# wagnva/semantic-nerf-for-satellite-data

Measured on AMD Instinct MI355X. Metric: train rays/sec (4096 rays x 64 samples), higher is better.
Workload: dtype f32(f16x2)

## Files before the change

semantic-nerf-for-satellite-data_amd/csrc/api.hip:

```cpp
#include <stdarg.h>
#include <stdio.h>
#include <stdlib.h>
#include <string.h>

#include <mutex>

#include "aux_kernels.h"
#include "bsp.h"
#include "composite.h"
#include "gemm.h"
#include "plan.h"

namespace snerf {

int forward_bsp(const Plan& p, const float* pk, const SnerfInputs* in, const SnerfOutputs* out, void* workspace, hipStream_t st);
int backward_bsp(const Plan& p, const float* pk, const SnerfInputs* in, const SnerfOutGrads* go, float* gp, float* d_t, float* d_t_s,
                 void* workspace, hipStream_t st);

static thread_local char g_err[512] = "";
void set_error(const char* fmt, ...) {
  va_list ap;
  va_start(ap, fmt);
  vsnprintf(g_err, sizeof(g_err), fmt, ap);
  va_end(ap);
// ... 182 lines not shown
  p.FA = p.Wf + p.Xp;
  int nb = 0;
  p.blk_rgb = nb++;
  p.blk_sem = sem ? nb++ : -1;
  p.blk_beta = nb++;
  p.blk_sbeta = sbeta ? nb++ : -1;
  p.blk_sun = nb++;
  p.nblk = nb;
  p.KF = (nb - 1) * p.H;
  p.KF = round_up(p.KF, 128);
  p.sun_col = p.KF;
  p.N1 = p.KF + p.H;

  size_t off = 0;
  auto take = [&](size_t n) { size_t o = off; off += round_up_sz(n, 64); return o; };
  for (int i = 0; i < p.L; ++i) {
    p.k_tr[i] = (i == 0) ? p.Ep : (((p.skip_mask >> i) & 1u) ? p.Ep + p.W : p.W);
    p.w_tr[i] = take((size_t)p.W * p.k_tr[i]);
    p.b_tr[i] = take(p.W);
  }
  p.w_fs = take((size_t)(p.W + NARROW) * p.W); p.b_fs = take(p.W + NARROW);
  p.w_h1 = take((size_t)p.N1 * p.FA); p.b_h1 = take(p.N1);
  p.w_s2 = take((size_t)p.H * p.H); p.b_s2 = take(p.H);
  p.w_s3 = take((size_t)p.H * p.H); p.b_s3 = take(p.H);
  p.w_s4 = take((size_t)NARROW * p.H); p.b_s4 = take(NARROW);
  p.w_fin = take((size_t)NARROW * p.KF); p.b_fin = take(NARROW);
  p.sky_floats = 9 * p.H + 4;
  p.sky = take(p.sky_floats);
  p.n_fp32 = off;
  {
    const char* ev = getenv("SNERF_COMPOSE_FEATS");
    p.compose_feats = p.pl == 2 && (p.H & 31) == 0 && p.N1 + NARROW <= 2048 && !(ev && ev[0] == '0' && ev[1] == 0);
  }
  if (!p.compose_feats) { plan_weights(p); plan_bsp(p); return SNERF_OK; }
  Plan q = p;
  q.compose_feats = false;
  plan_weights(q);
  plan_bsp(q);
  plan_weights(p);
  plan_bsp(p);
  if (q.packed_floats > p.packed_floats) p.packed_floats = q.packed_floats;
  if (q.ws_bytes > p.ws_bytes) p.ws_bytes = q.ws_bytes;
  return SNERF_OK;
}

struct TableBuilder {
  CopyTable tabs[4];
  int nt = 0;
  bool missing = false;
  TableBuilder() { memset(tabs, 0, sizeof(tabs)); nt = 1; }
  void add(float* user, int user_ld, int rows, int cols, size_t dst_off, int dst_ld) {
    if (!user) { missing = true; return; }
    if (tabs[nt - 1].n == COPY_TABLE_MAX) ++nt;
    CopyEntry& e = tabs[nt - 1].e[tabs[nt - 1].n++];
    e.user = user; e.user_ld = user_ld; e.rows = rows; e.cols = cols; e.dst_off = dst_off; e.dst_ld = dst_ld;
  }
};

static void build_tables(const Plan& p, const SnerfParams* w, TableBuilder& tb) {
  const int W = p.W, H = p.H, E = p.E;
  for (int i = 0; i < p.L; ++i) {
    const bool skip = (p.skip_mask >> i) & 1u;
    if (i == 0) {
      tb.add(w->fc_w[0], E, W, E, p.w_tr[0], p.k_tr[0]);
    } else if (skip) {
      tb.add(w->fc_w[i], E + W, W, E, p.w_tr[i], p.k_tr[i]);
// ... 256 lines not shown
```

semantic-nerf-for-satellite-data_amd/csrc/aux_kernels.h:

```cpp
#pragma once
#include "common.h"
#include "../../include/snerf_hip.h"

namespace snerf {

struct EncodeArgs {
  const float* rays = nullptr;
  const float* xyz = nullptr;
  const float* z = nullptr;
  const float* sun_d = nullptr; int sun_stride = 3;
  const float* t = nullptr; const float* t_s = nullptr;
  int dir_is_sun = 0;
  int N = 0, S = 0, F = 0, Ep = 0;
  int FA = 0, W = 0, Xp = 0, x_sun = 0, x_t = 3, x_ts = -1, tau = 0;
  unsigned* zero = nullptr; int zero_n = 0;
};

struct CopyEntry {
  float* user; int user_ld; int rows; int cols; unsigned long long dst_off; int dst_ld;
};
constexpr int COPY_TABLE_MAX = 40;
struct CopyTable { CopyEntry e[COPY_TABLE_MAX]; int n; };

int launch_zero_bytes(void* p, size_t bytes, hipStream_t st);
int launch_sample_z(const float* rays, const float* zsteps, const float* u, float* z, int N, int S, hipStream_t st);
int launch_copy_table(const CopyTable& tb, float* packed, int mode, hipStream_t st);
int launch_reduce_rows(const float* in, int n_in, size_t in_stride, int width, float* out, size_t out_stride,
                       int group, int accumulate, hipStream_t st);
int reduce_partials(const float* in, int n_in, size_t in_stride, int width, float* tmp, float* out, hipStream_t st);
struct RedJob { const float* in; float* out; unsigned long long stride; long long width; int n_in; int blk0; int vec; int cols; int in_ld; int out_ld; int store; int pad; };
constexpr int RED_MAX = 56;
struct RedTable { RedJob j[RED_MAX]; int n = 0; int blocks = 0; };
constexpr int RED_CHUNK = 24;
struct RedChunk { RedJob j[RED_CHUNK]; int n = 0; };
int red_add_elem(RedTable& tb, const float* in, int n_in, size_t stride, size_t width, float* out);
int red_add_elem2d(RedTable& tb, const float* in, int n_in, size_t stride, int rows, int cols, int in_ld, float* out, int out_ld);
int red_add_col(RedTable& tb, const float* in, int n_in, size_t stride, int width, float* out);
int red_store_last(RedTable& tb);
int launch_reductions(const RedTable& elem, const RedTable& col, hipStream_t st);
int launch_ray_sum32(const float* d32, int col0, int N, int S, int tau, float* out, hipStream_t st);
int launch_embedding_rows(const float* table, int n_embed, int tau, const long long* idx, int n, float* rows, hipStream_t st);
int launch_embedding_backward(const long long* idx, const float* d_rows, int n, int tau, int n_embed, float* grad, hipStream_t st);

}
```

semantic-nerf-for-satellite-data_amd/csrc/bsp.h:

```cpp
#pragma once
#include "common.h"
#include "gemm.h"

namespace snerf {
namespace bsp {

constexpr int RB = 128;
constexpr int CB = 128;
constexpr int E_MAX = 100;
constexpr int E_QUIET = 60;

typedef __amdgpu_buffer_rsrc_t srd_t;
typedef unsigned int u32x4 __attribute__((ext_vector_type(4)));
typedef unsigned int u32x2 __attribute__((ext_vector_type(2)));
typedef _Float16 f16x8 __attribute__((ext_vector_type(8)));
typedef _Float16 f16x4 __attribute__((ext_vector_type(4)));
constexpr unsigned OOB = 0xFFFFFFF0u;

__host__ __device__ inline int ncb_of(int ld) { return (ld + CB - 1) / CB; }
__host__ __device__ inline size_t plane_bytes(size_t rows, int ld, int pl = 2) { return rows * (size_t)ld * 2 * pl; }
__host__ __device__ inline size_t etab_ints(size_t rows, int ld) { return ((rows + RB - 1) / RB) * (size_t)ncb_of(ld); }
__host__ __device__ inline unsigned g16_off(int k, int pl = 2) { return (unsigned)(k >> 4) * 32u * (unsigned)pl + (unsigned)(k & 15) * 2u; }

__host__ __device__ inline int exp_of_maxbits(unsigned b) {
// ... 45 lines not shown
}

__device__ __forceinline__ void sum8(const u32x4 hi, const u32x4 lo, float (&x)[8]) {
#pragma unroll
  for (int i = 0; i < 4; ++i) {
    asm("v_fma_mix_f32 %0, %1, 1.0, %2 op_sel_hi:[1,0,1]" : "=v"(x[2 * i]) : "v"(hi[i]), "v"(lo[i]));
    asm("v_fma_mix_f32 %0, %1, 1.0, %2 op_sel:[1,0,1] op_sel_hi:[1,0,1]" : "=v"(x[2 * i + 1]) : "v"(hi[i]), "v"(lo[i]));
  }
}
__device__ __forceinline__ void cvt8f(const u32x4 hi, float (&x)[8]) {
  const f16x8 h = __builtin_bit_cast(f16x8, hi);
#pragma unroll
  for (int i = 0; i < 8; ++i) x[i] = (float)h[i];
}

__host__ __device__ inline int wf16_row(int m) { return (m & 0x13) | ((m & 4) << 1) | ((m & 8) >> 1); }

struct KcArgs {
  const char* A = nullptr; const int* EA = nullptr; int lda = 0; int a_col0 = 0;
  const char* A2 = nullptr; const int* EA2 = nullptr; int lda2 = 0; int a2_col0 = 0;
  int Ka = 0;
  const char* W = nullptr;
  const int* EW = nullptr;
  int w_rb32 = 0, w_row0 = 0, w_k0 = 0; unsigned w_bytes = 0;
  int I = 0, J = 0, K = 0;
  char* C = nullptr; int* EC = nullptr; int ldc = 0; int c_col0 = 0;
  float* Cf = nullptr;
  const float* bias = nullptr;
  int act = ACT_NONE; float w0 = 1.f;
  unsigned* Csign = nullptr;
  int aux_mode = AUX_NONE;
  const char* H = nullptr; const int* EH = nullptr; int ldh = 0; int h_col0 = 0; const unsigned* Hsign = nullptr;
  float* colsum = nullptr; int ldcs = 0;
  int tiles_i = 0, tiles_j = 0;
  int tj_skip = -1;
  int tiles_jr = 0;
  int rev = 0;
  int dbg = 0;
  int* tile_ctr = nullptr;
  int pl = 2;
  const float* nd_w = nullptr; float* nd_out = nullptr; unsigned long long nd_stride = 0;
  int nd_omax = 0, nd_ldw = 0;
  int nd_rows[8] = {0, 0, 0, 0, 0, 0, 0, 0}, nd_row0[8] = {0, 0, 0, 0, 0, 0, 0, 0}, nd_woff[8] = {0, 0, 0, 0, 0, 0, 0, 0};
};
__host__ __device__ inline size_t sign_words(size_t rows, int ld) { return ((rows + 31) / 32) * (size_t)((ld + 63) / 64) * 64; }

struct DwArgs {
  const char* A = nullptr; const int* EA = nullptr; int lda = 0; int a_col0 = 0;
  const char* B = nullptr; const int* EB = nullptr; int ldb = 0; int b_col0 = 0;
  int I = 0, J = 0, P = 0;
  float* C = nullptr; int ldc = 0;
  int k_split = 0, n_split = 1; unsigned long long slab_stride = 0;
  int tiles_i = 0, tiles_j = 0;
  int pl = 2;
};

constexpr int TR_MAXL = 8;
constexpr int TR_SLOTS = TR_MAXL + 1;
struct TrunkArgs {
  const char* pe = nullptr; const int* Epe = nullptr;
  int P = 0, W = 0, L = 0; unsigned skip_mask = 0;
  int gamma_free_layer = 0;
  const char* Wp[TR_SLOTS] = {}; const int* EW[TR_SLOTS] = {}; unsigned w_bytes[TR_SLOTS] = {}; int K[TR_SLOTS] = {};
  const float* bias[TR_SLOTS] = {}; float w0[TR_SLOTS] = {};
  char* F = nullptr; int* EF = nullptr; int ldf = 0;
  char* H[TR_MAXL] = {}; int* EH[TR_MAXL] = {}; unsigned* Hsign[TR_MAXL] = {};
// ... 69 lines not shown
```

semantic-nerf-for-satellite-data_amd/csrc/bsp_aux.hip:

```cpp
#include "bsp.h"
#include "aux_kernels.h"

namespace snerf {
namespace bsp {

__device__ __forceinline__ float block_max_256(float m, float* sm) {
#pragma unroll
  for (int o = 32; o >= 1; o >>= 1) m = fmaxf(m, __shfl_xor(m, o, 64));
  __syncthreads();
  if ((threadIdx.x & 63) == 0) sm[threadIdx.x >> 6] = m;
  __syncthreads();
  return fmaxf(fmaxf(sm[0], sm[1]), fmaxf(sm[2], sm[3]));
}

__global__ __launch_bounds__(256) void to_planes_kernel(const float* __restrict__ src, int ld_src, int rows, int cols,
                                                        char* __restrict__ dst, int* __restrict__ E, int ld, int col0, int pl) {
  __shared__ float sm[4];
  const int rb = blockIdx.y, cb = blockIdx.x;
  const int t = threadIdx.x, c8 = cb * 128 + (t & 15) * 8;
  float v[8][8];
  float m = 0.f;
#pragma unroll
  for (int i = 0; i < 8; ++i) {
    const int r = rb * 128 + (t >> 4) + 16 * i;
// ... 402 lines not shown
    float4 tsum = make_float4(0.f, 0.f, 0.f, 0.f);
#pragma unroll
    for (int i = 0; i < 32; ++i) { const float4 q = sm[i][threadIdx.x]; tsum.x += q.x; tsum.y += q.y; tsum.z += q.z; tsum.w += q.w; }
    *reinterpret_cast<float4*>(partial + (size_t)blockIdx.x * 32 + 4 * threadIdx.x) = tsum;
  }
  if (pl == nullptr) return;
  int e[2];
#pragma unroll
  for (int h = 0; h < 2; ++h) {
    e[h] = exp_of_maxbits(__float_as_uint(smx[0][h]));
    if (threadIdx.x == 0 && r0 + 128 * h < rows) E[(r0 >> 7) + h] = e[h];
  }
#pragma unroll
  for (int i = 0; i < 8; ++i) {
    const int r = r0 + rg + 32 * i;
    if (r >= rows) continue;
    const float sc = pow2f(e[i >> 2]);
    const float x[4] = {v[i].x * sc, v[i].y * sc, v[i].z * sc, v[i].w * sc};
    f16x4 h, l;
#pragma unroll
    for (int c = 0; c < 4; ++c) { h[c] = (_Float16)x[c]; l[c] = (_Float16)(x[c] - (float)h[c]); }
    char* d = pl + (size_t)r * 64 * npl + g16_off(4 * c4, npl);
    *reinterpret_cast<f16x4*>(d) = h;
    if (npl == 2) *reinterpret_cast<f16x4*>(d + 32) = l;
  }
}

int launch_colsum32_bsp(const float* in, int rows, float* partial, char* planes, int* E, int pl, hipStream_t st) {
  hipLaunchKernelGGL(colsum32_bsp_kernel, dim3((rows + 255) / 256), dim3(256), 0, st, in, rows, partial, planes, E, pl);
  SNERF_LAUNCH_CHECK();
  return SNERF_OK;
}

}
}
```

semantic-nerf-for-satellite-data_amd/csrc/bsp_kc.hip:

```cpp
#include "bsp_kc_epi.h"

namespace snerf {
namespace bsp {

constexpr int KC_A = 128 * 128, KC_RING = 3;
constexpr int KC_RINGB = KC_RING * KC_A;
constexpr int KC_XREG = KC_RINGB;
constexpr int KC_BIAS = KC_XREG + 4 * 4096;
constexpr int KC_ETAB = KC_BIAS + 2 * 1024;
constexpr int KC_SMAX = KC_ETAB + 2 * 512;
constexpr int KC_NEXT = KC_SMAX + 64;
constexpr int KC_HSIGN = KC_NEXT + 64;
constexpr int KC_LDS = KC_HSIGN + 4 * 1024;
constexpr int KC_NDW = KC_HSIGN;
constexpr int KC_NDW_FLOATS = 2560;
constexpr int KC_LDS_ND = KC_NDW + 4 * KC_NDW_FLOATS;
template <int PL, int ACT, int AUX, bool COLSUM, bool SIGNS, int SINM, bool DIAG = false, int NDOT = 0>
__global__ __launch_bounds__(256, 2) void gemm_kc_kernel(const KcArgs) {
  const kargs_t p = kargs();
  __shared__ __attribute__((aligned(16))) char lds[NDOT > 0 ? KC_LDS_ND : KC_LDS];
  float* smax = reinterpret_cast<float*>(lds + KC_SMAX);
  const int t = threadIdx.x, lane = t & 63;
  const int wave = __builtin_amdgcn_readfirstlane(t >> 6);
  const int wj0 = wave * 64;
// ... 482 lines not shown
                const unsigned rs = __float_as_uint(root) | ((sword[mi] << (31 - (16 * nj + 8 * gg + c))) & 0x80000000u);
                v[c] *= __uint_as_float(rs);
              }
            } else if (AUX == AUX_RELU_MASK) {
              float hv[8];
              cvt8f(hh[gg], hv);
#pragma unroll
              for (int c = 0; c < 8; ++c) v[c] = hv[c] > 0.f ? v[c] : 0.f;
            }
#pragma unroll
            for (int c = 0; c < 8; ++c) {
              if (COLSUM) cs[8 * gg + c] += v[c];
              acc[mi][nj][8 * gg + c] = v[c];
            }
            if (jw + 16 * gq < e->J) {
              const float m8 = absmax3(v[6], v[7], absmax3(v[4], v[5], absmax3(v[2], v[3], absmax3(v[0], v[1], 0.f))));
              wmax = fmaxf(wmax, (BIAS && (32 * mi + pt) >= nrows) ? 0.f : m8);
            }
          }
        }
        if (COLSUM && e->colsum != nullptr) {
#pragma unroll
          for (int r = 0; r < 16; ++r) cs[r] = sum32(cs[r]);
          if ((el & 31) == 31) {
#pragma unroll
            for (int gg = 0; gg < 2; ++gg)
              if (jw + 16 * (2 * nj + gg) < e->J) {
                float* d = e->colsum + (size_t)c_ti * e->ldcs + jw + 16 * (2 * nj + gg) + 8 * lh;
                *reinterpret_cast<float4*>(d) = make_float4(cs[8 * gg] * fac, cs[8 * gg + 1] * fac, cs[8 * gg + 2] * fac, cs[8 * gg + 3] * fac);
                *reinterpret_cast<float4*>(d + 4) = make_float4(cs[8 * gg + 4] * fac, cs[8 * gg + 5] * fac, cs[8 * gg + 6] * fac, cs[8 * gg + 7] * fac);
              }
          }
        }
      }
      constexpr bool RAW = AUX != AUX_NONE || COLSUM;
      wmax = wave_max(wmax) * (RAW ? fac : 1.f);
      if (el == 0) smax[wave] = wmax;
      barrier_raw();
      const float bmax = fmaxf(smax[wave & 2], smax[(wave & 2) + 1]);
      const int eC = exp_of_maxbits(__float_as_uint(bmax));
      const float sc = pow2f(eC) * (RAW ? fac : 1.f);
      if ((wave & 1) == 0 && el == 0 && wave_cols) e->EC[(size_t)c_ti * ncb_of(e->ldc) + ((e->c_col0 + jw) >> 7)] = eC;
      if (more) headW();
#pragma unroll
      for (int mi = 0; mi < 4; ++mi) {
        u32x4 ph1[4];
#pragma unroll
        for (int nj = 0; nj < 2; ++nj) {
          u32x4 phi[2], plo[2];
#pragma unroll
          for (int gg = 0; gg < 2; ++gg) {
            float v[8];
#pragma unroll
            for (int c = 0; c < 8; ++c) v[c] = acc[mi][nj][8 * gg + c];
            if constexpr (PL == 2) {
              split8(v, sc, phi[gg], plo[gg]);
              strip_put(gg, phi[gg], plo[gg]);
            } else {
              cvt8(v, sc, ph1[2 * nj + gg]);
              strip_put1(nj, gg, ph1[2 * nj + gg]);
            }
          }
          if constexpr (PL == 2) {
            strip_flush(mi, nj);
            keep_planes(phi, plo);
          }
        }
        if constexpr (PL == 1) {
          strip_flush(mi, 0);
          keep_planes1(ph1);
        }
      }
    }
    if (!more) break;
    vb = vbn;
    first = false;
  }
}

int prof_hook_begin(double flops, int variant, hipStream_t st);
void prof_hook_end(int token, hipStream_t st);
int check_kc(const KcArgs& a, bool narrow);

static int g_kc_grid_override = 0;
void kc_set_grid_override(int n) { g_kc_grid_override = n > 0 ? n : 0; }
static int kc_slots() {
  if (g_kc_grid_override > 0) return g_kc_grid_override;
  static const int n = [] {
    int dev = 0, cus = 256;
    if (hipGetDevice(&dev) != hipSuccess || hipDeviceGetAttribute(&cus, hipDeviceAttributeMultiprocessorCount, dev) != hipSuccess || cus <= 0) cus = 256;
    return 2 * cus;
  }();
  return n;
}

static bool cs_bias_check(const KcArgs& a) {
  if (a.colsum != nullptr && a.bias != nullptr) { set_error("bsp gemm: bias and column sums in one launch"); return true; }
  return false;
}

int launch_kc(const KcArgs& a0, hipStream_t st) {
  KcArgs a = a0;
  if (!a.A2) { a.A2 = a.A; a.EA2 = a.EA; a.lda2 = a.lda; a.a2_col0 = a.a_col0; if (a.Ka == 0) a.Ka = a.K; }
  int rc = check_kc(a, false);
  if (rc) return rc;
  if (cs_bias_check(a)) return SNERF_ERR_BAD_DESC;
  a.tiles_i = (a.I + 127) / 128;
  a.tiles_jr = (a.J + 255) / 256;
  if (a.tj_skip >= a.tiles_jr || (a.tj_skip >= 0 && a.tiles_jr < 2)) { set_error("bsp gemm: tj_skip beyond the column tiles"); return SNERF_ERR_BAD_DESC; }
  a.tiles_j = a.tiles_jr - (a.tj_skip >= 0 ? 1 : 0);
  if (a.nd_w != nullptr) {
    if (a.nd_omax == 0) { a.nd_omax = 1; a.nd_ldw = 0; for (int tj = 0; tj < 8; ++tj) { a.nd_rows[tj] = tj < a.tiles_jr ? 1 : 0; a.nd_row0[tj] = 0; } }
    int off = 0;
    for (int tj = 0; tj < a.tiles_jr && tj < 8; ++tj) { a.nd_woff[tj] = off; off += 256 * a.nd_rows[tj]; }
    if (a.tiles_jr > 8 || off > KC_NDW_FLOATS || (a.nd_omax != 1 && a.nd_omax != 5)) { set_error("bsp gemm: folded projections beyond the LDS table"); return SNERF_ERR_BAD_DESC; }
    for (int tj = 0; tj < a.tiles_jr; ++tj) if (a.nd_rows[tj] > a.nd_omax) { set_error("bsp gemm: nd_rows > nd_omax"); return SNERF_ERR_BAD_DESC; }
  }
#ifdef KC_DIAG_BUILD
  constexpr bool DIAG = true;
  static const int dbg = [] { const char* e = getenv("SNERF_KC_DBG"); return e ? atoi(e) : 0; }();
  a.dbg = dbg;
  if (dbg & 2) a.w_bytes = 0;
#else
  constexpr bool DIAG = false;
#endif
  const int ntiles = a.tiles_i * a.tiles_j, slots = kc_slots();
  const dim3 grid(ntiles < slots ? ntiles : slots), block(256);
  const int tok = prof_hook_begin(2.0 * a.I * (double)a.J * a.K, 0, st);
  const bool cs = a.colsum != nullptr;
#define KC_LAUNCH(ACT_, AUX_, CS_, SG_, SM_) do { if (a.pl == 2) hipLaunchKernelGGL((gemm_kc_kernel<2, ACT_, AUX_, CS_, SG_, SM_, DIAG>), grid, block, 0, st, a); \
// ... 24 lines not shown
```

semantic-nerf-for-satellite-data_amd/csrc/bsp_pass.hip:

```cpp
#include "aux_kernels.h"
#include "bsp.h"
#include "composite.h"
#include "normals.h"
#include "plan.h"

namespace snerf {

namespace {
struct Ws {
  char* base;
  char* c(size_t off) const { return base + off; }
  float* f(size_t off) const { return reinterpret_cast<float*>(base + off); }
  int* i(size_t off) const { return reinterpret_cast<int*>(base + off); }
  unsigned* u(size_t off) const { return reinterpret_cast<unsigned*>(base + off); }
  void a(bsp::KcArgs& g, const PlaneT& t, int k, int col0 = 0) const { g.A = c(t.o); g.EA = i(t.e); g.lda = t.ld; g.a_col0 = col0; g.Ka = k; }
  void a2(bsp::KcArgs& g, const PlaneT& t) const { g.A2 = c(t.o); g.EA2 = i(t.e); g.lda2 = t.ld; }
  void out(bsp::KcArgs& g, const PlaneT& t, int col0 = 0) const { g.C = c(t.o); g.EC = i(t.e); g.ldc = t.ld; g.c_col0 = col0; g.Csign = t.s ? u(t.s) : nullptr; }
  void h(bsp::KcArgs& g, const PlaneT& t, int col0 = 0) const { g.H = c(t.o); g.EH = i(t.e); g.ldh = t.ld; g.h_col0 = col0; g.Hsign = t.s ? u(t.s) : nullptr; }
  void dz(bsp::DwArgs& g, const PlaneT& t) const { g.A = c(t.o); g.EA = i(t.e); g.lda = t.ld; g.a_col0 = 0; }
  void x(bsp::DwArgs& g, const PlaneT& t, int col0) const { g.B = c(t.o); g.EB = i(t.e); g.ldb = t.ld; g.b_col0 = col0; }
};
struct WOp { const char* W; const int* EW; int rb32; unsigned bytes; int K; };
WOp wop(const Plan& p, const float* pk, int job) {
  const char* planes = reinterpret_cast<const char*>(pk + p.n_fp32);
// ... 245 lines not shown
    g.k_split = m.sp.k_split; g.n_split = m.sp.ns; g.slab_stride = m.stride; g.pl = p.pl;
    return bsp::launch_dw(g, narrow_i, st);
  };
  auto dw_reduce = [&](const DwMat& m, size_t count, float* gout) { return red_add_elem(rq.elem, m.slab, m.sp.ns, m.stride, count, gout); };
  auto narrow_grad = [&](const float* dnar, float* part, const PlaneT& t, float* gout) {
    RC(bsp::launch_colsum32_bsp(dnar, P, part, ws.c(t.o), ws.i(t.e), p.pl, st));
    return red_add_col(rq.col, part, (P + 255) / 256, NARROW, NARROW, gout);
  };
  float* dsig = ws.f(p.o_dsig); float* dfin = ws.f(p.o_dfin); float* dsun = ws.f(p.o_dsun);
  if (embed && p.sc) {
    if (d_t) RC(launch_zero_bytes(d_t, (size_t)p.N * p.tau * sizeof(float), st));
    if (d_t_s && p.x_ts >= 0) RC(launch_zero_bytes(d_t_s, (size_t)p.N * p.tau * sizeof(float), st));
    return SNERF_OK;
  }
  CompBwdArgs b;
  CompArgs& c = b.f;
  c.N = p.N; c.S = p.S; c.H = H; c.C = p.C; c.sc = p.sc; c.sem_sigmoid = p.sem_sigmoid; c.has_sbeta = p.blk_sbeta >= 0;
  c.z = ws.f(p.o_z); c.sigo = ws.f(p.o_sigo); c.fino = ws.f(p.o_fino); c.suno = ws.f(p.o_suno);
  narrow_parts(c, p, pk, ws);
  c.sun_d = in->sun_d; c.sun_stride = in->sun_stride; c.sky = pk + p.sky;
  b.T = ws.f(p.o_T); b.rgbraw = ws.f(p.o_rgbraw);
  b.g_rgb = go->rgb; b.g_depth = go->depth; b.g_weights = go->weights; b.g_transparency = go->transparency;
  b.g_albedo = go->albedo; b.g_sun = go->sun; b.g_sky = go->sky; b.g_beta = go->beta; b.g_sigmas = go->sigmas;
  b.g_beta_s = go->beta_semantic; b.g_logits = go->semantic_logits;
  b.d_sigo = dsig; b.d_fino = dfin; b.d_suno = dsun; b.sky_slab = (p.sc || embed) ? nullptr : ws.f(p.o_skyslab);
  b.zero = ws.u(p.o_kcq); b.zero_n = KCQ_SLOTS * 16;
  RC(launch_composite_bwd(b, st));
  if (!p.sc && !embed)
    RC(red_add_col(rq.col, ws.f(p.o_skyslab), p.comp_blocks * 4, (size_t)p.sky_floats, p.sky_floats, gp + p.sky));


  const PlaneT dz1 = p.dza.view(p.h1w);
  const int sun_col = p.sc ? 0 : p.sun_col;
  if (!p.sc) {
    if (embed) RC(bsp::launch_colsum32_bsp(dfin, P, r.nar_fin, ws.c(p.pdfin.o), ws.i(p.pdfin.e), p.pl, st));
    else {
      RC(narrow_grad(dfin, r.nar_fin, p.pdfin, gp + p.b_fin));
      RC(dw_gemm(r.w_fin, p.pdfin, NARROW, true, p.h1, 0, p.KF));
      RC(dw_reduce(r.w_fin, (size_t)NARROW * p.KF, gp + p.w_fin));
    }
    bsp::KcArgs g;
    ws.a(g, p.pdfin, NARROW); weights(g, p, pk, p.wj_tfin);
    g.I = P; g.J = p.KF; g.K = NARROW; ws.out(g, dz1);
    dact(g, p.h1);
    colsum(g, r.cs_fin, p.KF);
    if (p.compose_feats) g.ldcs = r.ld_cs1;
    RC(launch_kc(g));
    if (!p.compose_feats && !embed) RC(bias_from_colsum(r.cs_fin, p.KF, gp + p.b_h1));
  }
  if (!embed) {
    RC(narrow_grad(dsun, r.nar_sun, p.pdsun, gp + p.b_s4));
    RC(dw_gemm(r.w_s4, p.pdsun, NARROW, true, p.s3, 0, H));
    RC(dw_reduce(r.w_s4, (size_t)NARROW * H, gp + p.w_s4));
    bsp::KcArgs g;
    ws.a(g, p.pdsun, NARROW); weights(g, p, pk, p.wj_ts4);
    g.I = P; g.J = H; g.K = NARROW; ws.out(g, p.dsa);
    dact(g, p.s3);
    colsum(g, r.cs_s3, H);
    RC(launch_kc(g));
    RC(bias_from_colsum(r.cs_s3, H, gp + p.b_s3));
    RC(dw_gemm(r.w_s3, p.dsa, H, false, p.s2, 0, H));
    RC(dw_reduce(r.w_s3, (size_t)H * H, gp + p.w_s3));
    ws.a(g, p.dsa, H); g.K = H; weights(g, p, pk, p.wj_ts3);
    ws.out(g, p.dsb);
    dact(g, p.s2);
    colsum(g, r.cs_s2, H);
    RC(launch_kc(g));
    RC(bias_from_colsum(r.cs_s2, H, gp + p.b_s2));
    RC(dw_gemm(r.w_s2, p.dsb, H, false, p.h1, sun_col, H));
    RC(dw_reduce(r.w_s2, (size_t)H * H, gp + p.w_s2));
    ws.a(g, p.dsb, H); weights(g, p, pk, p.wj_ts2);
    ws.out(g, dz1, sun_col);
    dact(g, p.h1, sun_col);
    colsum(g, r.cs_sun, H);
    if (p.compose_feats) g.ldcs = r.ld_cs1;
    RC(launch_kc(g));
    if (!p.compose_feats) RC(bias_from_colsum(r.cs_sun, H, gp + p.b_h1 + (size_t)p.sun_col));
  }
  auto transient_grads = [&]() {
    const bool want_t = d_t != nullptr, want_ts = d_t_s != nullptr && p.x_ts >= 0;
    if (p.sc) {
      if (want_t) RC(launch_zero_bytes(d_t, (size_t)p.N * p.tau * sizeof(float), st));
      if (want_ts) RC(launch_zero_bytes(d_t_s, (size_t)p.N * p.tau * sizeof(float), st));
    } else if (want_t || want_ts) {
      int b_lo = p.blk_beta, b_hi = p.blk_beta;
      auto use = [&](int blk, bool on) { if (on && blk >= 0) { if (blk < b_lo) b_lo = blk; if (blk > b_hi) b_hi = blk; } };
      use(p.blk_rgb, p.rgb_t); use(p.blk_sem, p.sem_t || p.sem_ts); use(p.blk_sbeta, true);
      const int k_lo = b_lo * H, k_n = (b_hi + 1 - b_lo) * H;
      float* dext = ws.f(p.o_dfin);
      bsp::KcArgs x;
      ws.a(x, dz1, k_n, k_lo); weights(x, p, pk, p.wj_th1, p.Wf, k_lo);
      x.I = P; x.J = p.Xp; x.K = k_n; x.Cf = dext;
      RC(bsp::launch_kc_narrow(x, st));
      if (want_t) RC(launch_ray_sum32(dext, p.x_t, p.N, p.S, p.tau, d_t, st));
      if (want_ts) RC(launch_ray_sum32(dext, p.x_ts, p.N, p.S, p.tau, d_t_s, st));
    }
    return (int)SNERF_OK;
  };
  if (embed) return transient_grads();
  PlaneT dz_cur = p.dza.view(W);
  PlaneT dz_nxt = p.dzb.view(W);
  const bool sig_live = !p.sc || go->weights != nullptr || go->transparency != nullptr || go->sigmas != nullptr;
  const PlaneT& hl = p.h[p.L - 1];
  bool uncompose = false;
  if (p.compose_feats) {
    const int r0 = p.sc ? p.sun_col : 0;
    const int nt = (P + 127) / 128, X = p.FA - W;
    RC(dw_gemm(r.w_h1, dz1, p.h1w, false, p.fa, 0, p.FA));
    RC(red_add_elem2d(rq.elem, r.w_h1.slab + W, r.w_h1.sp.ns, r.w_h1.stride, p.h1w, X, p.FA, gp + p.w_h1 + (size_t)r0 * p.FA + W, p.FA));
    RC(red_add_elem2d(rq.elem, r.w_h1.slab, r.w_h1.sp.ns, r.w_h1.stride, p.h1w, W, p.FA, r.w_h1.slab, p.FA));
    RC(red_store_last(rq.elem));
    RC(red_add_col(rq.col, r.cs_fin, nt, (size_t)r.ld_cs1, p.h1w, r.cs_fin));
    RC(red_store_last(rq.col));
    uncompose = true;
    RC(transient_grads());
    if (sig_live) {
      RC(narrow_grad(dsig, r.nar_sig, p.pdsig, gp + p.b_fs + W));
      RC(dw_gemm(r.w_fs, p.pdsig, NARROW, true, hl, 0, W));
      RC(dw_reduce(r.w_fs, (size_t)NARROW * W, gp + p.w_fs + (size_t)W * W));
    }
    { const PlaneT sw = dz_cur; dz_cur = dz_nxt; dz_nxt = sw; }
    bsp::KcArgs g;
    ws.a(g, dz1, p.h1w);
    if (sig_live) ws.a2(g, p.pdsig);
    weights(g, p, pk, p.wj_th1, 0, r0); g.I = P; g.J = W; g.K = sig_live ? p.h1w + NARROW : p.h1w;
    ws.out(g, dz_cur);
    dact(g, hl, 0, (p.L == 1) ? 30.f : 1.f);
    colsum(g, r.cs_hl, W);
    RC(launch_kc(g));
    RC(bias_from_colsum(r.cs_hl, W, gp + p.b_tr[p.L - 1]));
  }
  const PlaneT dfa = p.dzb.view(p.FA);
  if (!p.compose_feats) {
    const int r0 = p.sc ? p.sun_col : 0;
    RC(dw_gemm(r.w_h1, dz1, p.h1w, false, p.fa, 0, p.FA));
    RC(dw_reduce(r.w_h1, (size_t)p.h1w * p.FA, gp + p.w_h1 + (size_t)r0 * p.FA));
    bsp::KcArgs g;
    ws.a(g, dz1, p.h1w); weights(g, p, pk, p.wj_th1, 0, r0);
    g.I = P; g.J = W; g.K = p.h1w; ws.out(g, dfa);
    colsum(g, r.cs_fa, p.FA);
    RC(launch_kc(g));
    RC(red_add_col(rq.col, r.cs_fa, (P + 127) / 128, (size_t)cs_ld(p.FA), W, gp + p.b_fs));
    RC(transient_grads());
  }
  if (!p.compose_feats) {
    if (sig_live) RC(narrow_grad(dsig, r.nar_sig, p.pdsig, gp + p.b_fs + W));
    RC(dw_gemm(r.w_fs, dfa, W, false, hl, 0, W));
    if (sig_live) RC(dw_gemm(r.w_fs, p.pdsig, NARROW, true, hl, 0, W, (size_t)W * W));
    RC(dw_reduce(r.w_fs, (size_t)(sig_live ? W + NARROW : W) * W, gp + p.w_fs));
    bsp::KcArgs g;
    ws.a(g, dfa, W);
    if (sig_live) ws.a2(g, p.pdsig);
    weights(g, p, pk, p.wj_tfs); g.I = P; g.J = W; g.K = sig_live ? W + NARROW : W;
    ws.out(g, dz_cur);
    dact(g, hl, 0, (p.L == 1) ? 30.f : 1.f);
    colsum(g, r.cs_hl, W);
    RC(launch_kc(g));
    RC(bias_from_colsum(r.cs_hl, W, gp + p.b_tr[p.L - 1]));
  }
  for (int i = p.L - 1; i >= 0; --i) {
    const BwdRegions::Layer& t = r.tr[i];
    if (i > 0 && ((p.skip_mask >> i) & 1u)) {
      RC(dw_gemm(t.w_gamma, dz_cur, W, false, p.pe, 0, p.Ep));
      RC(dw_gemm(t.w, dz_cur, W, false, p.h[i - 1], 0, W));
      RC(red_add_elem2d(rq.elem, t.w_gamma.slab, t.w_gamma.sp.ns, t.w_gamma.stride, W, p.Ep, p.Ep, gp + p.w_tr[i], p.k_tr[i]));
      RC(red_add_elem2d(rq.elem, t.w.slab, t.w.sp.ns, t.w.stride, W, W, W, gp + p.w_tr[i] + p.Ep, p.k_tr[i]));
    } else {
      if (i == 0) RC(dw_gemm(t.w, dz_cur, W, false, p.pe, 0, p.Ep));
      else RC(dw_gemm(t.w, dz_cur, W, false, p.h[i - 1], 0, W));
      RC(dw_reduce(t.w, (size_t)W * p.k_tr[i], gp + p.w_tr[i]));
    }
    if (i == 0) break;
    bsp::KcArgs g;
    ws.a(g, dz_cur, W); weights(g, p, pk, p.wj_tt[i]);
    g.I = P; g.J = W; g.K = W; ws.out(g, dz_nxt);
    dact(g, p.h[i - 1], 0, (i - 1 == 0) ? 30.f : 1.f);
// ... 80 lines not shown
```

semantic-nerf-for-satellite-data_amd/csrc/plan.h:

```cpp
#pragma once
#include "bsp.h"
#include "common.h"
#include "../../include/snerf_hip.h"

namespace snerf {

constexpr int NARROW = 32;
constexpr int MAX_CLASSES = 16;
constexpr int ND_FIN = 5;
constexpr int MAX_SKY_UNITS = 8;

struct PlaneT { size_t o = 0, e = 0, s = 0; int ld = 0; };
struct PlaneScratch {
  size_t o = 0, e = 0; int maxw = 0;
  PlaneT view(int ld) const { PlaneT t; t.o = o; t.e = e; t.ld = ld; return t; }
};

struct Plan {
  int N = 0, S = 0, P = 0, Pp = 0;
  int W = 0, H = 0, L = 0, E = 0, Ep = 0, F = 0, tau = 0, C = 0;
  bool siren = false, train = false, sc = false, sem_sigmoid = false;
  bool relight = false;
  bool embed_grad = false;
  bool geometry = false;
// ... 14 lines not shown
  size_t w_h1 = 0, b_h1 = 0;
  size_t w_s2 = 0, b_s2 = 0, w_s3 = 0, b_s3 = 0;
  size_t w_s4 = 0, b_s4 = 0;
  size_t w_fin = 0, b_fin = 0;
  size_t sky = 0;
  int sky_floats = 0;
  size_t n_fp32 = 0;
  size_t packed_floats = 0;
  int pl = 2;

  size_t o_z = 0, o_T = 0, o_rgbraw = 0;
  PlaneT pe, fa, h1, s2, s3, h[SNERF_MAX_LAYERS];
  size_t o_sigo = 0, o_fino = 0, o_suno = 0;
  size_t o_sigpart = 0, o_sunpart = 0, o_finpart = 0;
  bool nd_sig = false, nd_sun = false;
  bool fuse_trunk = false;
  bool nd_fin = false;
  PlaneScratch dza, dzb;
  PlaneT dsa, dsb, pdsig, pdfin, pdsun;
  size_t o_dsig = 0, o_dfin = 0, o_dsun = 0;
  size_t o_skyslab = 0;
  size_t o_kcq = 0;
  size_t o_rq = 0, rq_floats = 0;
  bsp::WPackTable wj = {};
  int wj_tr[SNERF_MAX_LAYERS] = {0}, wj_tt[SNERF_MAX_LAYERS] = {0};
  int wj_fs = 0, wj_sig = 0, wj_tfs = 0, wj_h1 = 0, wj_th1 = 0, wj_s2 = 0, wj_ts2 = 0, wj_s3 = 0, wj_ts3 = 0, wj_s4 = 0, wj_ts4 = 0,
      wj_fin = 0, wj_tfin = 0;
  size_t wp_bytes = 0;
  int h1w = 0;
  bool compose_feats = false;
  int wj_first = 0;
  size_t o_wc = 0;
  size_t o_bc = 0;
  int comp_blocks = 0;
  size_t ws_bytes = 0;
};

inline bool skips_beta_block(const Plan& p, bool want_beta) {
  return p.nd_fin && !p.train && p.H == 256 && p.blk_beta >= 0 && !want_beta && !p.rgb_t && p.blk_sbeta < 0;
}

constexpr int KCQ_SLOTS = 64;
struct DwSplit { int ns = 1; int k_split = 32; };
DwSplit dw_choose_bsp(int P, int rows, int cols, bool narrow_rows);

#define RC(expr) do { int _rc = (expr); if (_rc) return _rc; } while (0)

int make_plan(const SnerfDesc* d, Plan* pl);

size_t bsp_rq_floats(const Plan& p);

}
```

Measured before the change: 170,000.

## Compute per-ray extras weight grads and transient grads from 64-row column sums

Since the extra input columns (sun direction, transient embeddings) are constant within each ray, the backward GEMM epilogue now also writes 64-row column sums of the h1 gradient. A new ray_extras kernel uses these sums to build the extras' weight-gradient slab and the d_t/d_t_s gradients. This lets the dW GEMM for the first head layer cover only W columns, and removes the separate transient-gradient GEMM over the full sample count. The cost is an extra epilogue store, a new kernel and stricter shape requirements (S divisible by 64, tau ≤ 16, Xp == 16).

```diff
diff --git a/semantic-nerf-for-satellite-data_amd/csrc/api.hip b/semantic-nerf-for-satellite-data_amd/csrc/api.hip
--- a/semantic-nerf-for-satellite-data_amd/csrc/api.hip
+++ b/semantic-nerf-for-satellite-data_amd/csrc/api.hip
@@ -238,6 +238,10 @@
     const char* ev = getenv("SNERF_COMPOSE_FEATS");
     p.compose_feats = p.pl == 2 && (p.H & 31) == 0 && p.N1 + NARROW <= 2048 && !(ev && ev[0] == '0' && ev[1] == 0);
   }
+  {
+    const char* ev = getenv("SNERF_RAY_EXTRAS");
+    p.ray_extras = p.compose_feats && p.train && p.S % 64 == 0 && ((p.N1 + 3) & ~3) <= 2048 && !(ev && ev[0] == '0' && ev[1] == 0);
+  }
   if (!p.compose_feats) { plan_weights(p); plan_bsp(p); return SNERF_OK; }
   Plan q = p;
   q.compose_feats = false;
diff --git a/semantic-nerf-for-satellite-data_amd/csrc/aux_kernels.h b/semantic-nerf-for-satellite-data_amd/csrc/aux_kernels.h
--- a/semantic-nerf-for-satellite-data_amd/csrc/aux_kernels.h
+++ b/semantic-nerf-for-satellite-data_amd/csrc/aux_kernels.h
@@ -42,4 +42,16 @@
 int launch_embedding_rows(const float* table, int n_embed, int tau, const long long* idx, int n, float* rows, hipStream_t st);
 int launch_embedding_backward(const long long* idx, const float* d_rows, int n, int tau, int n_embed, float* grad, hipStream_t st);
 
+struct RayExtrasArgs {
+  EncodeArgs a;
+  const float* cs64 = nullptr; int ldcs = 0; int G = 0;
+  int rows = 0;
+  float* slab = nullptr; unsigned long long slab_stride = 0; int ldw = 0, col0 = 0, k_split = 0, n_split = 0, n_jb = 0;
+  const float* w = nullptr; int ldw_w = 0, k_lo = 0, k_n = 0;
+  float* d_t = nullptr; float* d_ts = nullptr;
+};
+namespace bsp {
+int launch_ray_extras(const RayExtrasArgs& g, hipStream_t st);
 }
+
+}
diff --git a/semantic-nerf-for-satellite-data_amd/csrc/bsp.h b/semantic-nerf-for-satellite-data_amd/csrc/bsp.h
--- a/semantic-nerf-for-satellite-data_amd/csrc/bsp.h
+++ b/semantic-nerf-for-satellite-data_amd/csrc/bsp.h
@@ -101,6 +101,7 @@
   int aux_mode = AUX_NONE;
   const char* H = nullptr; const int* EH = nullptr; int ldh = 0; int h_col0 = 0; const unsigned* Hsign = nullptr;
   float* colsum = nullptr; int ldcs = 0;
+  float* colsum64 = nullptr; int ldcs64 = 0;
   int tiles_i = 0, tiles_j = 0;
   int tj_skip = -1;
   int tiles_jr = 0;
diff --git a/semantic-nerf-for-satellite-data_amd/csrc/bsp_aux.hip b/semantic-nerf-for-satellite-data_amd/csrc/bsp_aux.hip
--- a/semantic-nerf-for-satellite-data_amd/csrc/bsp_aux.hip
+++ b/semantic-nerf-for-satellite-data_amd/csrc/bsp_aux.hip
@@ -458,5 +458,117 @@
   return SNERF_OK;
 }
 
-}
-}
+constexpr int RX_RAYS = 256;
+__device__ __forceinline__ const float* extras_column(const EncodeArgs& a, int c, int& stride) {
+  if (c >= a.x_sun && c < a.x_sun + 3) { stride = a.sun_stride; return a.sun_d + (c - a.x_sun); }
+  if (a.t != nullptr && c >= a.x_t && c < a.x_t + a.tau) { stride = a.tau; return a.t + (c - a.x_t); }
+  if (a.t_s != nullptr && a.x_ts >= 0 && c >= a.x_ts && c < a.x_ts + a.tau) { stride = a.tau; return a.t_s + (c - a.x_ts); }
+  stride = 0;
+  return nullptr;
+}
+__global__ __launch_bounds__(256) void ray_extras_kernel(const RayExtrasArgs g) {
+  __shared__ float xs[RX_RAYS][16];
+  __shared__ float part[4][16][64];
+  const EncodeArgs& a = g.a;
+  const int t = threadIdx.x, wave = __builtin_amdgcn_readfirstlane(t >> 6), lane = t & 63;
+  const int n_slab = g.slab != nullptr ? g.n_jb * g.n_split : 0;
+  if ((int)blockIdx.x < n_slab) {
+    const int q = (int)blockIdx.x / g.n_jb, j = ((int)blockIdx.x - q * g.n_jb) * 64 + lane;
+    const int g0 = q * (g.k_split >> 6);
+    const int g1 = min(g.G, g0 + (g.k_split >> 6));
+    const int n0 = (int)(((long long)g0 * 64) / a.S);
+    const int nr = g1 > g0 ? min(RX_RAYS, (int)(((long long)(g1 - 1) * 64) / a.S) - n0 + 1) : 0;
+    int xstride = 0;
+    const float* const xcol = extras_column(a, t & 15, xstride);
+#pragma unroll 4
+    for (int r = t >> 4; r < nr; r += 16) xs[r][t & 15] = (xcol != nullptr && n0 + r < a.N) ? xcol[(size_t)(n0 + r) * xstride] : 0.f;
+    __syncthreads();
+    float acc[16];
+#pragma unroll
+    for (int c = 0; c < 16; ++c) acc[c] = 0.f;
+    if (j < g.rows) {
+      const int gpr = a.S >> 6;
+      for (int gb = g0 + wave; gb < g1; gb += 32) {
+        float v[8];
+#pragma unroll
+        for (int u = 0; u < 8; ++u) v[u] = gb + 4 * u < g1 ? g.cs64[(size_t)(gb + 4 * u) * g.ldcs + j] : 0.f;
+#pragma unroll
+        for (int u = 0; u < 8; ++u) {
+          const int r = (gb + 4 * u) / gpr - n0;
+          if (gb + 4 * u < g1 && r >= 0 && r < nr) {
+#pragma unroll
+            for (int c = 0; c < 16; ++c) acc[c] = fmaf(v[u], xs[r][c], acc[c]);
+          }
+        }
+      }
+    }
+#pragma unroll
+    for (int c = 0; c < 16; ++c) part[wave][c][lane] = acc[c];
+    __syncthreads();
+    const int jj = t >> 2, c4 = (t & 3) * 4, jo = ((int)blockIdx.x - q * g.n_jb) * 64 + jj;
+    if (jo < g.rows) {
+      float o[4];
+#pragma unroll
+      for (int c = 0; c < 4; ++c) o[c] = ((part[0][c4 + c][jj] + part[1][c4 + c][jj]) + part[2][c4 + c][jj]) + part[3][c4 + c][jj];
+      *reinterpret_cast<float4*>(g.slab + (size_t)q * g.slab_stride + (size_t)jo * g.ldw + g.col0 + c4) = make_float4(o[0], o[1], o[2], o[3]);
+    }
+    return;
+  }
+  const int n = ((int)blockIdx.x - n_slab) * 4 + wave;
+  if (n >= a.N || (g.d_t == nullptr && g.d_ts == nullptr)) return;
+  const int gpr = a.S >> 6;
+  float acc[32];
+#pragma unroll
+  for (int c = 0; c < 32; ++c) acc[c] = 0.f;
+  for (int j = g.k_lo + lane; j < g.k_lo + g.k_n && j < g.rows; j += 64) {
+    float s = 0.f;
+    for (int h = 0; h < gpr; ++h) {
+      const int gi = n * gpr + h;
+      if (gi < g.G) s += g.cs64[(size_t)gi * g.ldcs + j];
+    }
+    const float* w = g.w + (size_t)j * g.ldw_w;
+#pragma unroll
+    for (int c = 0; c < 16; ++c)
+      if (c < a.tau) {
+        if (g.d_t != nullptr) acc[c] = fmaf(s, w[a.x_t + c], acc[c]);
+        if (g.d_ts != nullptr) acc[16 + c] = fmaf(s, w[a.x_ts + c], acc[16 + c]);
+      }
+  }
+#pragma unroll
+  for (int c = 0; c < 32; ++c)
+    if ((c & 15) < a.tau && ((c < 16) ? g.d_t != nullptr : g.d_ts != nullptr)) {
+      float v = acc[c];
+#pragma unroll
+      for (int o = 32; o >= 1; o >>= 1) v += __shfl_xor(v, o, 64);
+      if (lane == 0) (c < 16 ? g.d_t : g.d_ts)[(size_t)n * a.tau + (c & 15)] = v;
+    }
+}
+
+int launch_ray_extras(const RayExtrasArgs& g, hipStream_t st) {
+  const EncodeArgs& a = g.a;
+  const bool slab = g.slab != nullptr, ray = g.d_t != nullptr || g.d_ts != nullptr;
+  if (!slab && !ray) return SNERF_OK;
+  if (!g.cs64 || a.N <= 0 || a.S < 64 || (a.S & 63) || g.G != (int)(((long long)a.N * a.S) >> 6) || g.rows <= 0 || g.ldcs < g.rows || !a.sun_d ||
+      a.tau < 1 || a.tau > 16 || a.Xp != 16) {
+    set_error("ray extras: 64-row sums need n_samples % 64 == 0 and [N S / 64][>= rows] sums");
+    return SNERF_ERR_BAD_DESC;
+  }
+  if (slab && (g.k_split < 64 || (g.k_split & 63) || g.k_split > 64 * RX_RAYS || g.n_split < 1 || (long long)g.n_split * g.k_split < (long long)a.N * a.S ||
+               g.n_jb != (g.rows + 63) / 64 || (g.ldw & 3) || (g.col0 & 3) || g.col0 + 16 > g.ldw || (g.slab_stride & 3) ||
+               g.slab_stride < (unsigned long long)g.rows * g.ldw || ((uintptr_t)g.slab & 15))) {
+    set_error("ray extras: slab layout (splits of whole 64-row groups, <= 16384 rows each, 16 columns inside the slab row)");
+    return SNERF_ERR_BAD_DESC;
+  }
+  if (ray && (!g.w || g.ldw_w < 16 || g.k_lo < 0 || g.k_n <= 0 || g.k_lo + g.k_n > g.rows || (g.d_t != nullptr && (a.x_t < 0 || a.x_t + a.tau > 16)) ||
+              (g.d_ts != nullptr && (a.x_ts < 0 || a.x_ts + a.tau > 16)))) {
+    set_error("ray extras: the transient columns must lie inside the weight rows, the reading rows inside the sums");
+    return SNERF_ERR_BAD_DESC;
+  }
+  const int blocks = (slab ? g.n_jb * g.n_split : 0) + (ray ? (a.N + 3) / 4 : 0);
+  hipLaunchKernelGGL(ray_extras_kernel, dim3(blocks), dim3(256), 0, st, g);
+  SNERF_LAUNCH_CHECK();
+  return SNERF_OK;
+}
+
+}
+}
diff --git a/semantic-nerf-for-satellite-data_amd/csrc/bsp_kc.hip b/semantic-nerf-for-satellite-data_amd/csrc/bsp_kc.hip
--- a/semantic-nerf-for-satellite-data_amd/csrc/bsp_kc.hip
+++ b/semantic-nerf-for-satellite-data_amd/csrc/bsp_kc.hip
@@ -538,6 +538,21 @@
               }
           }
         }
+        if (COLSUM && e->colsum64 != nullptr) {
+#pragma unroll
+          for (int half = 0; half < 2; ++half)
+#pragma unroll
+            for (int gg = 0; gg < 2; ++gg) {
+              float h8[8];
+#pragma unroll
+              for (int c = 0; c < 8; ++c) h8[c] = sum32(acc[2 * half][nj][8 * gg + c] + acc[2 * half + 1][nj][8 * gg + c]) * fac;
+              if ((el & 31) == 31 && jw + 16 * (2 * nj + gg) < e->J) {
+                float* d = e->colsum64 + (size_t)(2 * c_ti + half) * e->ldcs64 + jw + 16 * (2 * nj + gg) + 8 * lh;
+                *reinterpret_cast<float4*>(d) = make_float4(h8[0], h8[1], h8[2], h8[3]);
+                *reinterpret_cast<float4*>(d + 4) = make_float4(h8[4], h8[5], h8[6], h8[7]);
+              }
+            }
+        }
       }
       constexpr bool RAW = AUX != AUX_NONE || COLSUM;
       wmax = wave_max(wmax) * (RAW ? fac : 1.f);
@@ -602,6 +617,10 @@
 
 static bool cs_bias_check(const KcArgs& a) {
   if (a.colsum != nullptr && a.bias != nullptr) { set_error("bsp gemm: bias and column sums in one launch"); return true; }
+  if (a.colsum64 != nullptr && (a.colsum == nullptr || a.act != ACT_NONE || a.ldcs64 < a.J || (a.ldcs64 & 3))) {
+    set_error("bsp gemm: 64-row column sums go with the 128-row ones, at a leading dimension >= J that is a multiple of 4");
+    return true;
+  }
   return false;
 }
 
diff --git a/semantic-nerf-for-satellite-data_amd/csrc/bsp_pass.hip b/semantic-nerf-for-satellite-data_amd/csrc/bsp_pass.hip
--- a/semantic-nerf-for-satellite-data_amd/csrc/bsp_pass.hip
+++ b/semantic-nerf-for-satellite-data_amd/csrc/bsp_pass.hip
@@ -301,6 +301,7 @@
 
   const PlaneT dz1 = p.dza.view(p.h1w);
   const int sun_col = p.sc ? 0 : p.sun_col;
+  float* const cs64 = p.ray_extras ? ws.f(p.o_dfin) : nullptr;
   if (!p.sc) {
     if (embed) RC(bsp::launch_colsum32_bsp(dfin, P, r.nar_fin, ws.c(p.pdfin.o), ws.i(p.pdfin.e), p.pl, st));
     else {
@@ -314,6 +315,7 @@
     dact(g, p.h1);
     colsum(g, r.cs_fin, p.KF);
     if (p.compose_feats) g.ldcs = r.ld_cs1;
+    if (p.ray_extras) { g.colsum64 = cs64; g.ldcs64 = r.ld_cs1; }
     RC(launch_kc(g));
     if (!p.compose_feats && !embed) RC(bias_from_colsum(r.cs_fin, p.KF, gp + p.b_h1));
   }
@@ -343,19 +345,37 @@
     dact(g, p.h1, sun_col);
     colsum(g, r.cs_sun, H);
     if (p.compose_feats) g.ldcs = r.ld_cs1;
+    if (p.ray_extras) { g.colsum64 = cs64 + sun_col; g.ldcs64 = r.ld_cs1; }
     RC(launch_kc(g));
     if (!p.compose_feats) RC(bias_from_colsum(r.cs_sun, H, gp + p.b_h1 + (size_t)p.sun_col));
   }
-  auto transient_grads = [&]() {
+  auto transient_grads = [&](bool slabs) {
     const bool want_t = d_t != nullptr, want_ts = d_t_s != nullptr && p.x_ts >= 0;
     if (p.sc) {
       if (want_t) RC(launch_zero_bytes(d_t, (size_t)p.N * p.tau * sizeof(float), st));
       if (want_ts) RC(launch_zero_bytes(d_t_s, (size_t)p.N * p.tau * sizeof(float), st));
-    } else if (want_t || want_ts) {
-      int b_lo = p.blk_beta, b_hi = p.blk_beta;
-      auto use = [&](int blk, bool on) { if (on && blk >= 0) { if (blk < b_lo) b_lo = blk; if (blk > b_hi) b_hi = blk; } };
-      use(p.blk_rgb, p.rgb_t); use(p.blk_sem, p.sem_t || p.sem_ts); use(p.blk_sbeta, true);
-      const int k_lo = b_lo * H, k_n = (b_hi + 1 - b_lo) * H;
+    }
+    const bool live = !p.sc && (want_t || want_ts);
+    int b_lo = p.blk_beta, b_hi = p.blk_beta;
+    auto use = [&](int blk, bool on) { if (on && blk >= 0) { if (blk < b_lo) b_lo = blk; if (blk > b_hi) b_hi = blk; } };
+    use(p.blk_rgb, p.rgb_t); use(p.blk_sem, p.sem_t || p.sem_ts); use(p.blk_sbeta, true);
+    const int k_lo = b_lo * H, k_n = (b_hi + 1 - b_lo) * H;
+    if (p.ray_extras) {
+      RayExtrasArgs x;
+      x.a.sun_d = in->sun_d; x.a.sun_stride = in->sun_stride; x.a.t = in->t; x.a.t_s = in->t_s;
+      x.a.N = p.N; x.a.S = p.S; x.a.tau = p.tau; x.a.FA = p.FA; x.a.Xp = p.Xp; x.a.x_sun = p.x_sun; x.a.x_t = p.x_t; x.a.x_ts = p.x_ts;
+      x.cs64 = cs64; x.ldcs = r.ld_cs1; x.G = P / 64; x.rows = p.h1w;
+      if (slabs) {
+        x.slab = r.w_h1.slab; x.slab_stride = r.w_h1.stride; x.ldw = r.w_h1.ldw; x.col0 = p.Wf;
+        x.k_split = r.w_h1.sp.k_split; x.n_split = r.w_h1.sp.ns; x.n_jb = (p.h1w + 63) / 64;
+      }
+      if (live) {
+        x.k_lo = k_lo; x.k_n = k_n; x.w = pk + p.w_h1 + p.Wf; x.ldw_w = p.FA;
+        x.d_t = d_t; x.d_ts = want_ts ? d_t_s : nullptr;
+      }
+      return bsp::launch_ray_extras(x, st);
+    }
+    if (live) {
       float* dext = ws.f(p.o_dfin);
       bsp::KcArgs x;
       ws.a(x, dz1, k_n, k_lo); weights(x, p, pk, p.wj_th1, p.Wf, k_lo);
@@ -366,7 +386,7 @@
     }
     return (int)SNERF_OK;
   };
-  if (embed) return transient_grads();
+  if (embed) return transient_grads(false);
   PlaneT dz_cur = p.dza.view(W);
   PlaneT dz_nxt = p.dzb.view(W);
   const bool sig_live = !p.sc || go->weights != nullptr || go->transparency != nullptr || go->sigmas != nullptr;
@@ -375,14 +395,15 @@
   if (p.compose_feats) {
     const int r0 = p.sc ? p.sun_col : 0;
     const int nt = (P + 127) / 128, X = p.FA - W;
-    RC(dw_gemm(r.w_h1, dz1, p.h1w, false, p.fa, 0, p.FA));
-    RC(red_add_elem2d(rq.elem, r.w_h1.slab + W, r.w_h1.sp.ns, r.w_h1.stride, p.h1w, X, p.FA, gp + p.w_h1 + (size_t)r0 * p.FA + W, p.FA));
+    RC(dw_gemm(r.w_h1, dz1, p.h1w, false, p.fa, 0, p.ray_extras ? W : p.FA));
+    if (p.ray_extras) RC(red_add_elem2d(rq.elem, r.w_h1.slab + p.Wf, r.w_h1.sp.ns, r.w_h1.stride, p.h1w, p.Xp, p.FA, gp + p.w_h1 + (size_t)r0 * p.FA + p.Wf, p.FA));
+    else RC(red_add_elem2d(rq.elem, r.w_h1.slab + W, r.w_h1.sp.ns, r.w_h1.stride, p.h1w, X, p.FA, gp + p.w_h1 + (size_t)r0 * p.FA + W, p.FA));
     RC(red_add_elem2d(rq.elem, r.w_h1.slab, r.w_h1.sp.ns, r.w_h1.stride, p.h1w, W, p.FA, r.w_h1.slab, p.FA));
     RC(red_store_last(rq.elem));
     RC(red_add_col(rq.col, r.cs_fin, nt, (size_t)r.ld_cs1, p.h1w, r.cs_fin));
     RC(red_store_last(rq.col));
     uncompose = true;
-    RC(transient_grads());
+    RC(transient_grads(true));
     if (sig_live) {
       RC(narrow_grad(dsig, r.nar_sig, p.pdsig, gp + p.b_fs + W));
       RC(dw_gemm(r.w_fs, p.pdsig, NARROW, true, hl, 0, W));
@@ -410,7 +431,7 @@
     colsum(g, r.cs_fa, p.FA);
     RC(launch_kc(g));
     RC(red_add_col(rq.col, r.cs_fa, (P + 127) / 128, (size_t)cs_ld(p.FA), W, gp + p.b_fs));
-    RC(transient_grads());
+    RC(transient_grads(false));
   }
   if (!p.compose_feats) {
     if (sig_live) RC(narrow_grad(dsig, r.nar_sig, p.pdsig, gp + p.b_fs + W));
diff --git a/semantic-nerf-for-satellite-data_amd/csrc/plan.h b/semantic-nerf-for-satellite-data_amd/csrc/plan.h
--- a/semantic-nerf-for-satellite-data_amd/csrc/plan.h
+++ b/semantic-nerf-for-satellite-data_amd/csrc/plan.h
@@ -70,6 +70,7 @@
   int wj_first = 0;
   size_t o_wc = 0;
   size_t o_bc = 0;
+  bool ray_extras = false;
   int comp_blocks = 0;
   size_t ws_bytes = 0;
 };
```

After: 170,600, median of 6. No clear change (+0.4%).
